# Storm-Tarran/LPR_381_Group_V22

Measured on AMD Instinct MI355X. Metric: simplex pivots/sec on 4096x8192 fp64 tableau; % HBM roofline, higher is better.
Workload: dtype f64

## Files before the change

### lpr_381_group_v22_amd/csrc/engine_common.hpp

```cpp
#pragma once

#include <hip/hip_runtime.h>

#include <cfloat>
#include <cstdint>
#include <cstdio>
#include <cstring>
#include <string>
#include <vector>

#include "../../include/lpr_engine.h"

#pragma clang fp contract(off)

namespace lpr {

constexpr int kWave = 64;
constexpr int kLdAlign = 16;
constexpr int32_t kRunning = -100;
constexpr int kMaxHeadGroups = 32;

void set_error(const char* fmt, ...);
const char* get_error();

#define LPR_HIP(expr)                                                                     \
    do {                                                                                  \
        hipError_t _e = (expr);                                                           \
        if (_e != hipSuccess) {                                                           \
            ::lpr::set_error("%s failed: %s (%s:%d)", #expr, hipGetErrorString(_e),       \
                             __FILE__, __LINE__);                                         \
            return LPR_DEVICE_ERROR;                                                      \
        }                                                                                 \
    } while (0)

// ... 117 lines not shown
    bool poisoned = false;
    hipGraphExec_t graph = nullptr;
    int graph_batch = 0;
    int graph_variant = -1;
    struct GraphKey {
        const void *T = nullptr, *T2 = nullptr, *log = nullptr, *basis = nullptr;
        const void *next_col = nullptr, *colbuf = nullptr;
        int rows = 0, cols = 0, ld = 0;
        bool operator==(const GraphKey& o) const {
            return T == o.T && T2 == o.T2 && log == o.log && basis == o.basis &&
                   next_col == o.next_col && colbuf == o.colbuf && rows == o.rows &&
                   cols == o.cols && ld == o.ld;
        }
    } graph_key;
    void* ov = nullptr;
    void* cut = nullptr;
    void* small = nullptr;
};

namespace lpr {
int tableau_reserve_rows(lpr_tableau* t, int rows_needed);
}
```

### lpr_381_group_v22_amd/csrc/lpr_engine.hip

```cpp
#include "engine_common.hpp"

#include <cmath>
#include <cstdlib>

#include <cstdarg>
#include <new>

#pragma clang fp contract(off)

namespace lpr {

static thread_local std::string g_err;

void set_error(const char* fmt, ...) {
    char buf[1024];
    va_list ap;
    va_start(ap, fmt);
    vsnprintf(buf, sizeof buf, fmt, ap);
    va_end(ap);
    g_err = buf;
}
const char* get_error() { return g_err.c_str(); }

void launch_select(lpr_tableau* t, int mode, int e_in, int r_in, int32_t* out_i);
// ... 24 lines not shown
int ov2_begin(lpr_tableau* t);
int ov2_launch_step(lpr_tableau* t, int K, int tr, int lp, int flags, hipEvent_t ev_start,
                    hipEvent_t ev_stop, int snap_slot);
int ov_read_stamps(lpr_tableau* t, uint64_t* out, int64_t cap, int64_t* count);
int ov2_join(lpr_tableau* t);
void ov_launch_sweep(lpr_tableau* t, int tr);
struct OvPoll {
    int32_t status, pending, kdone, cur, error;
    int64_t applied;
    double z[2];
};
int ov_poll(lpr_tableau* t, int parity, bool with_flags, OvPoll* out);
int ov_snapshot(lpr_tableau* t, int slot);
int ov_snapshot_wait(lpr_tableau* t, int slot, OvPoll* out);
void ov_adopt_buffer(lpr_tableau* t, int cur);
void rev_orphan(lpr_revised* s);
void bb_orphan(lpr_bb* b);
void sens_orphan(lpr_sens* s);
void comm_orphan(lpr_comm* c);
void knap_orphan(lpr_knap* k);
void batch_orphan(lpr_batch* b);
void bb_batch_orphan(lpr_bb_batch* b);
void sens_batch_orphan(lpr_sens_batch* b);
void cut_batch_orphan(lpr_cut_batch* b);
void knap_batch_orphan(lpr_knap_batch* b);
void rev_batch_orphan(lpr_rev_batch* b);
}
void lpr_cut_release(lpr_tableau* t);
namespace lpr {

// ... 135 lines not shown
    return t->graph && t->graph_batch == batch && t->graph_variant == variant &&
           t->graph_key == graph_key_now(t);
}

static void graph_stamp(lpr_tableau* t, int batch, int variant) {
    t->graph_batch = batch;
    t->graph_variant = variant;
    t->graph_key = graph_key_now(t);
}

static void release_device(lpr_tableau* t) {
    hipSetDevice(t->eng->device);
    if (t->eng->stream) hipStreamSynchronize(t->eng->stream);
    drop_graph(t);
    lpr_cut_release(t);
    ov_release(t);
    small_release(t);
    for (hipEvent_t ev : t->ev) hipEventDestroy(ev);
    t->ev.clear();
    hipFree(t->T);
    hipFree(t->T2);
    hipFree(t->rowbuf);
    hipFree(t->colbuf);
    hipFree(t->next_col);
    hipFree(t->next_rhs);
    hipFree(t->zparts);
    hipFree(t->basis);
    hipFree(t->log);
    hipFree(t->state);
    hipFree(t->scratch_i);
// ... 425 lines not shown
                if (q != hipErrorNotReady) LPR_HIP(q);
                (void)hipGetLastError();
            }
        }
        rc = drain();
        if (rc != LPR_OK_OPTIMAL) return rc;
    }
    ov_adopt_buffer(t, pl.cur);
    t->total_pivots = applied;
    res->status = status;
    res->block = K;
    res->pivots = applied - start_iter;
    res->total_pivots = applied;
    res->z = pl.z[applied & 1];
    return status;
}

}

using namespace lpr;

#define LPR_LIVE(t)                                                              \
    do {                                                                         \
        if (!(t) || !(t)->eng) {                                                 \
            set_error("tableau handle is null or its engine has been closed");   \
            return LPR_BAD_ARGUMENT;                                             \
        }                                                                        \
        if ((t)->poisoned) {                                                     \
            set_error("tableau handle is unusable: an earlier solve ended in a " \
                      "device-side hand-off timeout");                           \
// ... 228 lines not shown
    if (ld) *ld = t->ld;
    return LPR_OK_OPTIMAL;
}


int lpr_primal_solve(lpr_tableau* t, const lpr_solve_opts* opts, lpr_solve_result* res) {
    LPR_LIVE(t);
    if (!t || !res) {
        set_error("lpr_primal_solve: null argument");
        return LPR_BAD_ARGUMENT;
    }
    lpr_solve_opts o;
    std::memset(&o, 0, sizeof o);
    if (opts) o = *opts;
    const int hflags = (o.variant >> 16) & 511;
    o.variant &= 0xffff;
    if ((o.variant & 0xff00) == 0x5000) o.variant = 0x3000 | (o.variant & 0xff);
    if ((o.variant & 0xff00) == 0x6000) o.variant = 0x4000 | (o.variant & 0xff);
    lpr_engine* e = t->eng;
    hipStream_t s = e->stream;
    LPR_HIP(hipSetDevice(e->device));

    if (use_small(t, o)) return solve_small(t, o, res);
    if (use_fused(t, o)) return solve_fused(t, o, res);
    {
        const int K = block_size(t, o);
        if (K > 1) {
            const size_t tbytes = (size_t)t->rows * t->ld * sizeof(double);
            const bool big = (o.variant & 0xff00) == 0 && tbytes > kOverlapBytes;
            bool two_streams = (o.variant & 0xff00) == 0x3000 || big;
            const int tr = (o.variant & 0xff00) ? (o.variant & 0xff) : 8;
            if (two_streams && ov_ensure(t, true) != LPR_OK_OPTIMAL) two_streams = false;
            return solve_overlapped(t, o, K, tr, two_streams, hflags, res);
        }
    }
    const int variant = (o.variant > 0 && o.variant < 0x7000) ? o.variant - 1 : default_variant(t);
    int batch = o.batch > 0 ? o.batch : default_batch(t);
    const bool timed = o.time_kernels != 0;
    const int64_t start_iter = t->total_pivots;
    const int64_t max_iter = o.max_pivots > 0 ? start_iter + o.max_pivots : 0;

    PivotState* hs = t->h_state;
    hs->status = kRunning;
    hs->iter = start_iter;
    hs->max_iter = max_iter;
    hs->log_cap = t->log_cap;
    LPR_HIP(hipMemcpyAsync(&t->state->status, &hs->status, sizeof(int32_t), hipMemcpyHostToDevice,
// ... 250 lines not shown
```

### lpr_381_group_v22_amd/csrc/overlap_kernels.hip

```cpp
#include "engine_common.hpp"
#include "select_common.hpp"

#include <new>

#include <hip/hip_ext.h>

#pragma clang fp contract(off)

#ifndef LPR_OV_DIAG
#define LPR_OV_DIAG 0
#endif

namespace lpr {

constexpr int kOvMax = 16;
constexpr int kOvNT = 256;
constexpr int kOvGroups = 64;
constexpr unsigned kOvSpinMax = 1u << 22;
constexpr int kOvDoneCopies = 32;
constexpr int kOvDoneStride = 1088;
constexpr size_t kOvFlagWords = (size_t)(kOvDoneCopies + 1) * kOvDoneStride;
#ifndef LPR_OV_TILE_ROWS
#define LPR_OV_TILE_ROWS 32
#endif
// ... 10 lines not shown
#endif
constexpr bool kOvWaveHandoff = LPR_OV_WAVE_HANDOFF != 0;
constexpr int kOvWPG = kOvNT / 64;
constexpr int kOvParts = kOvGroups * kOvWPG;

struct OvCtl {
    int32_t status;
    int32_t pending;
    int32_t kdone;
    int32_t slot;
    int32_t cur;
    int32_t sweep;
    int32_t r[kOvMax];
    int32_t error;
    int32_t head_xcc;
    int64_t staged;
    int64_t applied;
    int64_t max_iter;
    int64_t log_cap;
};

struct OvBuffers {
    double* Tb[2];
    double* prow;
    double* fcol;
    double* zrow;
    double* bvec;
    ZPart* zparts;
    double* rparts;
    unsigned long long* gran;
    unsigned long long* xgran;
    unsigned long long* hx;
    unsigned* tileq;
    unsigned* sflag;
    unsigned long long* dbg;
    OvCtl* ctl;
    unsigned* bar;
    int32_t* basis;
    int32_t* log;
};

constexpr int kOvStampsPerPivot = 12;
constexpr int kOvStampPivots = 64;
constexpr size_t kOvDbgLaunch = (size_t)kOvStampPivots * kOvStampsPerPivot + 8;
constexpr size_t kOvDbgWords = kOvDbgLaunch + 64;

__global__ __launch_bounds__(1024) void k_ov_prologue(const double* __restrict__ T, int ld, int R,
                                                      int C, double* __restrict__ zrow,
                                                      double* __restrict__ bvec0,
                                                      ZPart* __restrict__ bank, int G,
                                                      unsigned long long* gbank,
                                                      unsigned epoch,
                                                      unsigned long long* gran_all,
                                                      unsigned long long* __restrict__ xgran,
                                                      unsigned* __restrict__ bar,
                                                      unsigned* __restrict__ tileq,
                                                      unsigned long long* __restrict__ hx,
                                                      unsigned* __restrict__ sflag) {
    __shared__ double lds_v[16];
    __shared__ int lds_i[16];
    const int tid = threadIdx.x, nt = blockDim.x;
    for (int k = tid; k < 9 * kOvParts; k += nt) gran_all[k] = 0ull;
    for (int k = tid; k < kOvGroups; k += nt) xgran[k] = 0ull;
    if (tid < 4) bar[tid] = 0u;
    if (tid < 2) tileq[tid] = 0u;
    if (tid == 0) *hx = 0ull;
    if (tid < 4) sflag[tid] = 0u;
    if (tid < kOvDoneCopies) sflag[(size_t)(tid + 1) * kOvDoneStride] = 0u;
    __syncthreads();
    Cand c;
    c.v = 0.0;
    c.i = -1;
    for (int j = tid; j < ld; j += nt) {
        const double v = T[j];
        zrow[j] = v;
        if (j < C - 1 && v < c.v) {
            c.v = v;
            c.i = j;
        }
    }
    c = block_cand_min(c, lds_v, lds_i);
    if (tid < G) {
        const double v = (tid == 0) ? c.v : 0.0;
        const int i = (tid == 0) ? c.i : -1;
        bank[tid].v = v;
        bank[tid].i = i;
    }
    const int nparts = kOvWaveHandoff ? G * kOvWPG : G;
    if (tid < nparts) {
        const double v = (tid == 0) ? c.v : 0.0;
        const int i = (tid == 0) ? c.i : -1;
        const unsigned long long e = (unsigned long long)epoch << 32;
        gbank[tid * 3 + 0] = e | (unsigned)__double2loint(v);
// ... 181 lines not shown
    __syncthreads();
    if (threadIdx.x == 0) {
        Cand r;
        r.v = lds_v[0];
        r.i = lds_i[0];
        for (int w = 1; w < (int)blockDim.x / kWave; ++w) {
            Cand o;
            o.v = lds_v[w];
            o.i = lds_i[w];
            r = cand_min(r, o);
        }
        gr_publish(g3, epoch, r.v, r.i, l2);
    }
}

template <int NT, bool STAMP>
__device__ void ov_heads(const OvBuffers B, int ld, int R, int C, int Rp, int K, int G, int lp,
                         bool solo, int spread, int no_l2, int wait_sweeps, int heads_done = -1) {
    if ((int)blockIdx.x % spread != 0) return;
    __shared__ double lds_v[16];
    __shared__ int lds_i[16];
    __shared__ int s_pick[2];
    const int tid = threadIdx.x, nt = blockDim.x;
    const int g = (int)blockIdx.x / spread;
    const bool lead = (g == 0);
    const OvCtl* ci = B.ctl + lp;
    OvCtl* co = B.ctl + (lp ^ 1);
    const int32_t status = ci->status;
    const int32_t pend_in = ci->pending;
    const int kb = solo ? 0 : ci->kdone;
    const int sa = ci->slot;
// ... 27 lines not shown
    double2* zrow2 = reinterpret_cast<double2*>(B.zrow);

    const int i_first = g * nt + tid, c2_first = g * nt + tid;
    const bool have_i = i_first < R, have_c = c2_first < ld2;
    double fA[kOvMax], myf[kOvMax];
    double2 pA[kOvMax], myp[kOvMax];
#pragma unroll
    for (int t = 0; t < kOvMax; ++t) {
        fA[t] = (t < kb && have_i) ? fcolA[(size_t)t * Rp + i_first] : 0.0;
        pA[t] = (t < kb && have_c) ? prowA2[(size_t)t * ld2 + c2_first] : make_double2(0.0, 0.0);
        myf[t] = 0.0;
        myp[t] = make_double2(0.0, 0.0);
    }
    double2 myz = have_c ? zrow2[c2_first] : make_double2(0.0, 0.0);
    double myb = have_i ? B.bvec[(size_t)(staged0 & 1) * Rp + i_first] : 0.0;
    const int lane = tid & (kWave - 1);
    const int rAv = (lane < kb) ? ci->r[lane] : -1;
    int rNv = -1;
    unsigned maskA = 0u, maskN = 0u;
#pragma unroll
    for (int t = 0; t < kOvMax; ++t) {
        const int rt = __builtin_amdgcn_readlane(rAv, t);
        maskA |= (have_i && rt == i_first) ? (1u << t) : 0u;
    }

    int32_t pend_out = pend_in;
    int32_t status_out = status;
    int count = 0;
    int err = 0;
    bool l2 = false;
// ... 84 lines not shown
                        s_pick[1] = fail;
                    }
                }
                __syncthreads();
                e = s_pick[0];
                if (s_pick[1]) {
                    err = 1;
                    break;
                }
            }
            OV_STAMP(q, 1);
            if (e < 0) {
                pend_out = LPR_OK_OPTIMAL;
                break;
            }
            double cq = have_i ? Tin[(size_t)i_first * ld + e] : 0.0;
            double pv = 0.0;
            if (lane < kb) pv = prowA[(size_t)lane * ld + e];
            else if (lane >= kOvMax && lane - kOvMax < q - 1)
                pv = xld(&prowN[(size_t)(lane - kOvMax) * ld + e]);
            if (STAMP) {
                __builtin_amdgcn_s_waitcnt(0);
                OV_STAMP(q, 2);
                OV_STAMP(q, 3);
            }
#pragma unroll
            for (int t = 0; t < kOvMax; ++t) {
                const double pt = ov_rl(pv, t);
                const double prod = fA[t] * pt;
                const double d = cq - prod;
                cq = ov_bitsel(maskA, t, pt, d);
            }
#pragma unroll
            for (int t = 0; t < kOvMax; ++t) {
                const double pt = ov_rl(pv, kOvMax + t);
                const double prod = myf[t] * pt;
                const double d = cq - prod;
                cq = ov_bitsel(maskN, t, pt, d);
            }
#pragma unroll
            for (int t = 0; t < kOvMax; ++t)
                if (t == q - 1) myf[t] = cq;
            Cand rc;
            rc.v = DBL_MAX;
            rc.i = -1;
            if (have_i) {
                hst(&colq[i_first], cq, l2);
                if (i_first >= 1 && cq > 1e-9) {
                    const double ratio = ieee_div(myb, cq);
                    if (ratio >= 0 && ratio < DBL_MAX) {
                        rc.v = ratio;
                        rc.i = i_first;
                    }
                }
            }
            for (int i = i_first + G * nt; i < R; i += G * nt) {
                double c = Tin[(size_t)i * ld + e];
#pragma unroll
                for (int t = 0; t < kOvMax; ++t) {
                    if (t < kb) {
// ... 7 lines not shown
                    }
                }
#pragma unroll
                for (int t = 0; t < kOvMax; ++t) {
                    if (t < q - 1) {
                        const double pt = ov_rl(pv, kOvMax + t);
                        if (i == __builtin_amdgcn_readlane(rNv, t)) {
                            c = pt;
                        } else {
                            const double prod = fcolN[(size_t)t * Rp + i] * pt;
                            c = c - prod;
                        }
                    }
                }
                hst(&colq[i], c, l2);
                if (c > 1e-9) {
                    const double ratio = ieee_div(bprev[i], c);
                    if (ratio >= 0 && ratio < rc.v) {
                        rc.v = ratio;
                        rc.i = i;
                    }
                }
            }
            OV_STAMP(q, 4);
            OV_STAMP(q, 5);
            int r;
            if (kOvWaveHandoff) {
                ov_publish_wave_min(rc, B.gran + ((size_t)2 * kOvParts + g * kOvWPG + tid / kWave) * 3,
                                    (unsigned)(2 * pidx + 2), l2);
                OV_STAMP(q, 6);
                int fail = 0;
                const Cand rr = gr_collect_waves(B.gran + (size_t)2 * 3 * kOvParts, G * kOvWPG,
                                                 (unsigned)(2 * pidx + 2), DBL_MAX, &fail);
                r = rr.i;
                if (fail) {
                    err = 1;
                    break;
                }
            } else {
                ov_publish_min(rc, lds_v, lds_i, B.gran + (size_t)(2 * kOvParts + g) * 3,
// ... 23 lines not shown
            if (mx > 0 && pidx >= mx) {
                pend_out = LPR_PIVOT_LIMIT;
                break;
            }

            double2 w = have_c ? Tin2[(size_t)r * ld2 + c2_first] : make_double2(0.0, 0.0);
            double fv = 0.0;
            {
                const double* src = nullptr;
                if (lane < kb) src = fcolA + (size_t)lane * Rp + r;
                else if (lane >= kOvMax && lane - kOvMax < q - 1)
                    src = fcolN + (size_t)(lane - kOvMax) * Rp + r;
                else if (lane == 32) src = bprev + r;
                else if (lane == 33) src = colq + r;
                else if (lane == 34) src = colq;
                if (src) fv = xld(src);
            }
            if (STAMP) {
                __builtin_amdgcn_s_waitcnt(0);
                OV_STAMP(q, 8);
            }
            const double wr = ov_rl(fv, 32);
            const double p = ov_rl(fv, 33);
            const double f0 = ov_rl(fv, 34);
            const unsigned ra = (unsigned)__ballot(lane < kb && rAv == r);
            const unsigned rn = (unsigned)__ballot(lane < q - 1 && rNv == r);
            if ((ra | rn) == 0u) {
#pragma unroll
                for (int t = 0; t < kOvMax; ++t) {
                    const double f = ov_rl(fv, t);
                    const double px = f * pA[t].x;
// ... 22 lines not shown
                        w.y = w.y - py;
                    }
                }
#pragma unroll
                for (int t = 0; t < kOvMax; ++t) {
                    if ((rn >> t) & 1u) {
                        w = myp[t];
                    } else {
                        const double f = ov_rl(fv, kOvMax + t);
                        const double px = f * myp[t].x;
                        const double py = f * myp[t].y;
                        w.x = w.x - px;
                        w.y = w.y - py;
                    }
                }
            }
            double dq[3];
            {
                const double dn[3] = {wr, w.x, w.y}, dd[3] = {p, p, p};
                ieee_div_n<3>(dn, dd, dq);
            }
            const double prhs = dq[0];
            if (lane == q - 1) rNv = r;
            if (have_i && i_first == r) maskN |= 1u << (q - 1);
            Cand n;
            n.v = 0.0;
            n.i = -1;
            if (have_c) {
                const int j = 2 * c2_first;
                double2 pq;
                pq.x = (j < C) ? dq[1] : 0.0;
                pq.y = (j + 1 < C) ? dq[2] : 0.0;
#pragma unroll
                for (int t = 0; t < kOvMax; ++t)
                    if (t == q - 1) myp[t] = pq;
                hst(&prowN[(size_t)(q - 1) * ld + j], pq.x, l2);
                hst(&prowN[(size_t)(q - 1) * ld + j + 1], pq.y, l2);
                const double mxp = f0 * pq.x;
                const double myp2 = f0 * pq.y;
                myz.x = myz.x - mxp;
                myz.y = myz.y - myp2;
                zrow2[c2_first] = myz;
                if (j < C - 1 && myz.x < n.v) {
                    n.v = myz.x;
                    n.i = j;
                }
                if (j + 1 < C - 1 && myz.y < n.v) {
                    n.v = myz.y;
                    n.i = j + 1;
                }
            }
            for (int c2 = c2_first + G * nt; c2 < ld2; c2 += G * nt) {
                double2 ww = Tin2[(size_t)r * ld2 + c2];
                double2 z = zrow2[c2];
#pragma unroll
                for (int t = 0; t < kOvMax; ++t) {
                    if (t < kb) {
                        const double2 ps = prowA2[(size_t)t * ld2 + c2];
                        if ((ra >> t) & 1u) {
                            ww = ps;
                        } else {
                            const double f = ov_rl(fv, t);
                            const double px = f * ps.x;
                            const double py = f * ps.y;
// ... 39 lines not shown
                    n.i = j + 1;
                }
            }
            if (have_i) {
                const double prod = cq * prhs;
                myb = (i_first == r) ? prhs : myb - prod;
                hst(&bnew[i_first], myb, l2);
            }
            for (int i = i_first + G * nt; i < R; i += G * nt) {
                const double prod = colq[i] * prhs;
                hst(&bnew[i], (i == r) ? prhs : bprev[i] - prod, l2);
            }
            OV_STAMP(q, 9);
            if (lead && tid == 0) {
                co->r[q - 1] = r;
                B.basis[r - 1] = e;
                if (pidx < log_cap) {
                    B.log[2 * pidx] = r;
                    B.log[2 * pidx + 1] = e;
                }
            }
            count = q;
            OV_STAMP(q, 10);
            if (kOvWaveHandoff)
                ov_publish_wave_min(n, B.gran + ((size_t)((pidx + 1) & 1) * kOvParts + g * kOvWPG +
                                                 tid / kWave) * 3,
                                    (unsigned)(2 * (pidx + 1) + 1), l2 && q < K);
            else
                ov_publish_min(n, lds_v, lds_i,
                               B.gran + ((size_t)((pidx + 1) & 1) * kOvParts + g) * 3,
                               (unsigned)(2 * (pidx + 1) + 1), l2 && q < K);
            OV_STAMP(q, 11);
        }
    }
#undef OV_STAMP
// ... 9 lines not shown
                    err = 1;
                    break;
                }
                __builtin_amdgcn_s_sleep(2);
            }
        }
        co->status = err ? LPR_DEVICE_ERROR : status_out;
        co->pending = pend_out;
        co->kdone = staged_now ? count : 0;
        co->slot = staged_now ? (sa ^ 1) : sa;
        co->staged = staged0 + (staged_now ? count : 0);
        co->max_iter = mx;
        co->log_cap = log_cap;
        co->error = err | ci->error;
        co->head_xcc = l2 ? (int)my_xcc : (staging ? -1 : ci->head_xcc);
        B.bar[lp ^ 1] = 0u;
        if (wait_sweeps >= 0) {
            const int ks = (status == kRunning) ? ci->kdone : 0;
            co->applied = ci->applied + ks;
            co->cur = (ks > 0) ? (ci->cur ^ 1) : ci->cur;
            co->sweep = ci->sweep ^ (ks > 0 ? 1 : 0);
        }
        if (solo) {
            B.tileq[1] = 0u;
            co->applied = ci->applied;
            co->cur = ci->cur;
            co->sweep = ci->sweep;
        }
    }
    if (heads_done >= 0) {
// ... 305 lines not shown
            co->applied = ci->applied + K;
            co->cur = (K > 0 && !INPLACE) ? (cur ^ 1) : cur;
            co->sweep = ci->sweep ^ (K > 0 ? 1 : 0);
        }
        B.tileq[lp ^ 1] = 0u;
        if (INPLACE) {
            co->status = ci->status;
            co->pending = ci->pending;
            co->kdone = 0;
            co->slot = ci->slot;
            co->staged = ci->staged;
            co->max_iter = ci->max_iter;
            co->log_cap = ci->log_cap;
            co->error = ci->error;
            co->head_xcc = ci->head_xcc;
            B.bar[lp ^ 1] = 0u;
        }
    }
    if (K <= 0) return;
    const int sa = ci->slot;
    const double* __restrict__ fc = fcol + (size_t)sa * kOvMax * Rp;
    const ov_v2d* __restrict__ prow2 =
        reinterpret_cast<const ov_v2d*>(prow + (size_t)sa * kOvMax * ld);
    if (static_tile >= 0) {
        ov_one_tile<TR, DB, INPLACE, TROWS>(B, ci, fc, prow2, static_tile, ld, R, Rp, K, cur);
        return;
    }
    const int ld2 = ld >> 1;
    const int nct = (ld2 + kOvNT - 1) / kOvNT, nrt = (R + TROWS - 1) / TROWS;
    const int ntiles = nct * nrt;
// ... 59 lines not shown
            const int pol = (at < ic_tiles ? 1 : 0) | (at >= ntiles - ic_tiles ? 2 : 0);
#define LPR_OV_HALF(P)                                                                             \
    ov_one_tile<TR, false, INPLACE, TROWS / 2, P>(B, ci, fc, prow2, tsplit + (u >> 1), ld, R, Rp, \
                                                  K, cur, TROWS, (u & 1) * (TROWS / 2))
            switch (pol) {
                case 1: LPR_OV_HALF(1); break;
                case 2: LPR_OV_HALF(2); break;
                case 3: LPR_OV_HALF(3); break;
                default: LPR_OV_HALF(0); break;
            }
#undef LPR_OV_HALF
        }
    }
}

template <int NT, bool STAMP>
__global__ __launch_bounds__(NT) void k_ov2_heads(const OvBuffers B, int ld, int R, int C, int Rp,
                                                  int K, int G, int lp, int spread, int no_l2,
                                                  int wait_sweeps, int heads_done) {
    ov_heads<NT, STAMP>(B, ld, R, C, Rp, K, G, lp, false, spread, no_l2, wait_sweeps, heads_done);
}

template <int TR, bool DB>
__global__ __launch_bounds__(kOvNT) void k_ov2_sweep(const OvBuffers B,
                                                     const double* __restrict__ fcol_ro,
                                                     const double* __restrict__ prow_ro, int ld,
                                                     int R, int Rp, int lp, int avoid,
                                                     int write_ctl, int sweeps_done,
                                                     int wait_heads, int hint_xcc, int ic_tiles,
                                                     int tall_pairs) {
    ov_tiles<TR, DB, false>(B, fcol_ro, prow_ro, ld, R, Rp, lp, -1, avoid, write_ctl != 0,
                            sweeps_done, wait_heads, hint_xcc, ic_tiles, tall_pairs);
}

template <int NT, bool STAMP>
__global__ __launch_bounds__(NT) void k_ov_heads(const OvBuffers B, int ld, int R, int C, int Rp,
                                                 int K, int G, int spread, int no_l2) {
    ov_heads<NT, STAMP>(B, ld, R, C, Rp, K, G, 0, true, spread, no_l2, -1);
}

template <int TR, bool DB, int TROWS = kOvTileRows>
__global__ __launch_bounds__(kOvNT) void k_ov_sweep(const OvBuffers B,
                                                    const double* __restrict__ fcol_ro,
                                                    const double* __restrict__ prow_ro, int ld,
                                                    int R, int Rp) {
    ov_tiles<TR, DB, true, TROWS>(B, fcol_ro, prow_ro, ld, R, Rp, 1, (int)blockIdx.x, 0);
}

}

#ifndef LPR_OV_KERNELS_ONLY

struct lpr_overlap_ctx {
    int rows = 0, ld = 0, Rp = 0;
    lpr::OvBuffers b{};
    lpr::OvCtl* h_ctl = nullptr;
    double* h_z = nullptr;
    double* T2 = nullptr;
    hipStream_t hstream = nullptr;
    hipEvent_t ev_h[2] = {nullptr, nullptr}, ev_s[2] = {nullptr, nullptr};
    int ev_idx = 0;
// ... 148 lines not shown
    std::memset(h, 0, 2 * sizeof(OvCtl));
    h[0].status = kRunning;
    h[0].pending = kRunning;
    h[0].staged = iter;
    h[0].applied = iter;
    h[0].max_iter = max_iter;
    h[0].log_cap = t->log_cap;
    h[0].head_xcc = -1;
    h[0].sweep = c->sweep_dir;
    h[1] = h[0];
    LPR_HIP(hipMemcpyAsync(c->b.ctl, h, 2 * sizeof(OvCtl), hipMemcpyHostToDevice, s));
    hipLaunchKernelGGL(k_ov_prologue, dim3(1), dim3(1024), 0, s, t->T, t->ld, t->rows, t->cols,
                       c->b.zrow, c->b.bvec + (size_t)(iter & 1) * c->Rp,
                       c->b.zparts + (iter & 1) * kOvGroups, ov_groups(t),
                       c->b.gran + (size_t)(iter & 1) * 3 * kOvParts, (unsigned)(2 * iter + 1),
                       c->b.gran, c->b.xgran, c->b.bar, c->b.tileq, c->b.hx, c->b.sflag);
    LPR_HIP(hipGetLastError());
    return LPR_OK_OPTIMAL;
}

int ov_set_log(lpr_tableau* t, int parity) {
    lpr_overlap_ctx* c = static_cast<lpr_overlap_ctx*>(t->ov);
    c->b.log = t->log;
    c->h_ctl[0].log_cap = t->log_cap;
    LPR_HIP(hipMemcpyAsync(&c->b.ctl[parity].log_cap, &c->h_ctl[0].log_cap, sizeof(int64_t),
                           hipMemcpyHostToDevice, t->eng->stream));
    LPR_HIP(hipStreamSynchronize(t->eng->stream));
    return LPR_OK_OPTIMAL;
}

void ov_launch_heads(lpr_tableau* t, int K, int flags) {
// ... 56 lines not shown
    const bool by_event = (flags & 32) == 0;
    const int wait_sweeps = by_event ? -1 : c->steps;
    const bool sweep_dev = (flags & 64) != 0 && !c->batch_first && c->steps >= 2 &&
                           c->head_xcc_hint >= 0 && snap_slot < 0;
    const int heads_done = (flags & 64) ? c->steps + 1 : -1;
    if (by_event) LPR_HIP(hipStreamWaitEvent(H, c->last_sweep, 0));
    if (!sweep_dev) LPR_HIP(hipStreamWaitEvent(S, c->ev_h[prev], 0));
    if (snap_slot >= 0) {
        LPR_HIP(hipMemcpyAsync(&c->h_snap[snap_slot], &c->b.ctl[lp], sizeof(OvCtl),
                               hipMemcpyDeviceToHost, S));
        LPR_HIP(hipEventRecord(c->ev_snap[snap_slot], S));
    }
    const int G = ov_groups(t);
    const int spread = ov_spread(G, flags);
    const int no_l2 = (flags & 6) ? 1 : 0;
    if (flags & 1)
        hipExtLaunchKernelGGL((k_ov2_heads<kOvNT, true>), dim3(G * spread), dim3(kOvNT), 0, H,
                              nullptr, c->ev_h[cur], 0, c->b, t->ld, t->rows, t->cols, c->Rp, K, G,
                              lp, spread, no_l2, wait_sweeps, heads_done);
    else
        hipExtLaunchKernelGGL((k_ov2_heads<kOvNT, false>), dim3(G * spread), dim3(kOvNT), 0, H,
                              nullptr, c->ev_h[cur], 0, c->b, t->ld, t->rows, t->cols, c->Rp, K, G,
                              lp, spread, no_l2, wait_sweeps, heads_done);
    const int nct = (t->ld / 2 + kOvNT - 1) / kOvNT;
    const int nrt = (t->rows + kOvTileRows - 1) / kOvTileRows;
    const dim3 grid(ov_sweep_grid(t, nct * nrt)), blk(kOvNT);
    const int avoid = (flags & (2 | 4 | 8)) ? 0 : ((flags & 16) ? 1 : 2);
    hipEvent_t sweep_done = ev_stop ? ev_stop : c->ev_s[cur];
    const int ic_tiles =
        (flags & 128) ? 0 : (int)(((size_t)kOvIcMB << 20) / ((size_t)kOvTileRows * kOvNT * 16));
    const int tall_pairs = (flags & 256) ? 0 : nrt * LPR_OV_TALL_PCT / 200;
// ... 87 lines not shown
        LPR_HIP(hipStreamSynchronize(t->eng->stream));
        LPR_HIP(hipMemcpy(out, c->b.dbg, (size_t)n * sizeof(uint64_t), hipMemcpyDeviceToHost));
    }
    return LPR_OK_OPTIMAL;
}

void ov_adopt_buffer(lpr_tableau* t, int cur) {
    lpr_overlap_ctx* c = static_cast<lpr_overlap_ctx*>(t->ov);
    if (cur == 1) {
        double* tmp = t->T;
        t->T = c->T2;
        c->T2 = tmp;
    }
}

}
#endif
```

Baseline: 98250.

## Run simplex on a condensed tableau that drops basic columns and uses spare slots

```diff
diff --git a/lpr_381_group_v22_amd/csrc/engine_common.hpp b/lpr_381_group_v22_amd/csrc/engine_common.hpp
--- a/lpr_381_group_v22_amd/csrc/engine_common.hpp
+++ b/lpr_381_group_v22_amd/csrc/engine_common.hpp
@@ -18,6 +18,8 @@
 constexpr int kWave = 64;
 constexpr int kLdAlign = 16;
 constexpr int32_t kRunning = -100;
+constexpr int32_t kOvLeaveNonFinite = -101;
+constexpr int32_t kOvLeaveSpares = -102;
 constexpr int kMaxHeadGroups = 32;
 
 void set_error(const char* fmt, ...);
@@ -165,6 +167,7 @@
         }
     } graph_key;
     void* ov = nullptr;
+    void* ovc = nullptr;
     void* cut = nullptr;
     void* small = nullptr;
 };
diff --git a/lpr_381_group_v22_amd/csrc/lpr_engine.hip b/lpr_381_group_v22_amd/csrc/lpr_engine.hip
--- a/lpr_381_group_v22_amd/csrc/lpr_engine.hip
+++ b/lpr_381_group_v22_amd/csrc/lpr_engine.hip
@@ -62,6 +62,14 @@
 int ov_snapshot(lpr_tableau* t, int slot);
 int ov_snapshot_wait(lpr_tableau* t, int slot, OvPoll* out);
 void ov_adopt_buffer(lpr_tableau* t, int cur);
+void ovc_release(lpr_tableau* t);
+bool ovc_fits(const lpr_tableau* t, int spares);
+int ovc_width(const lpr_tableau* t, int spares);
+int ovc_ensure(lpr_tableau* t, int spares);
+int ovc_condense(lpr_tableau* t, bool* ok);
+void ovc_enter(lpr_tableau* t);
+void ovc_leave(lpr_tableau* t);
+int ovc_expand(lpr_tableau* t);
 void rev_orphan(lpr_revised* s);
 void bb_orphan(lpr_bb* b);
 void sens_orphan(lpr_sens* s);
@@ -227,6 +235,7 @@
     if (t->eng->stream) hipStreamSynchronize(t->eng->stream);
     drop_graph(t);
     lpr_cut_release(t);
+    ovc_release(t);
     ov_release(t);
     small_release(t);
     for (hipEvent_t ev : t->ev) hipEventDestroy(ev);
@@ -682,6 +691,61 @@
     res->total_pivots = applied;
     res->z = pl.z[applied & 1];
     return status;
+}
+
+static constexpr int64_t kOvcMinPivots = 1024;
+
+static int ovc_spares(const lpr_tableau* t) {
+    if (const char* sp = std::getenv("LPR_TEST_OV_SPARES")) {
+        const long v = std::strtol(sp, nullptr, 10);
+        if (v >= 1 && v <= 4096) return (int)v;
+    }
+    const int s = (t->rows - 1) / 8 - 1;
+    return s < 1 ? 1 : s;
+}
+
+static bool use_condensed(const lpr_tableau* t, const lpr_solve_opts& o, int cflags, int hflags) {
+    if (cflags & 1) return false;
+    if (hflags & (1 | 32 | 64)) return false;
+    const int S = ovc_spares(t);
+    if (!ovc_fits(t, S)) return false;
+    if (cflags & 2) return true;
+    if (o.max_pivots > 0 && o.max_pivots < kOvcMinPivots) return false;
+    return ovc_width(t, S) < t->ld;
+}
+
+static int solve_condensed(lpr_tableau* t, const lpr_solve_opts& o, int K, int tr, int hflags,
+                           lpr_solve_result* res) {
+    const int64_t first = t->total_pivots;
+    lpr_solve_opts oc = o;
+    for (;;) {
+        const int64_t done = t->total_pivots - first;
+        if (o.max_pivots > 0) oc.max_pivots = o.max_pivots - done;
+        bool ok = false;
+        int rc = ovc_ensure(t, ovc_spares(t));
+        if (rc == LPR_OK_OPTIMAL) rc = ovc_condense(t, &ok);
+        if (rc != LPR_OK_OPTIMAL && rc != LPR_OUT_OF_MEMORY) return rc;
+        int status;
+        if (rc != LPR_OK_OPTIMAL || !ok) {
+            status = solve_overlapped(t, oc, K, tr, true, hflags, res);
+        } else {
+            ovc_enter(t);
+            status = solve_overlapped(t, oc, K, tr, true, hflags, res);
+            ovc_leave(t);
+            if (status == LPR_DEVICE_ERROR || status == LPR_OUT_OF_MEMORY ||
+                status == LPR_BAD_ARGUMENT)
+                return status;
+            rc = ovc_expand(t);
+            if (rc != LPR_OK_OPTIMAL) return rc;
+            if (status == kOvLeaveSpares) continue;
+            if (status == kOvLeaveNonFinite) {
+                if (o.max_pivots > 0) oc.max_pivots = o.max_pivots - (t->total_pivots - first);
+                status = solve_overlapped(t, oc, K, tr, true, hflags, res);
+            }
+        }
+        res->pivots = t->total_pivots - first;
+        return status;
+    }
 }
 
 }
@@ -940,6 +1004,7 @@
     std::memset(&o, 0, sizeof o);
     if (opts) o = *opts;
     const int hflags = (o.variant >> 16) & 511;
+    const int cflags = (o.variant >> 25) & 3;
     o.variant &= 0xffff;
     if ((o.variant & 0xff00) == 0x5000) o.variant = 0x3000 | (o.variant & 0xff);
     if ((o.variant & 0xff00) == 0x6000) o.variant = 0x4000 | (o.variant & 0xff);
@@ -957,6 +1022,13 @@
             bool two_streams = (o.variant & 0xff00) == 0x3000 || big;
             const int tr = (o.variant & 0xff00) ? (o.variant & 0xff) : 8;
             if (two_streams && ov_ensure(t, true) != LPR_OK_OPTIMAL) two_streams = false;
+            if (two_streams && (big || (cflags & 2)) && !(cflags & 1) &&
+                ovc_fits(t, ovc_spares(t)) && ovc_width(t, ovc_spares(t)) < t->ld) {
+                const int er = ovc_ensure(t, ovc_spares(t));
+                if (er != LPR_OK_OPTIMAL && er != LPR_OUT_OF_MEMORY) return er;
+            }
+            if (two_streams && use_condensed(t, o, cflags, hflags))
+                return solve_condensed(t, o, K, tr, hflags, res);
             return solve_overlapped(t, o, K, tr, two_streams, hflags, res);
         }
     }
diff --git a/lpr_381_group_v22_amd/csrc/overlap_kernels.hip b/lpr_381_group_v22_amd/csrc/overlap_kernels.hip
--- a/lpr_381_group_v22_amd/csrc/overlap_kernels.hip
+++ b/lpr_381_group_v22_amd/csrc/overlap_kernels.hip
@@ -48,6 +48,8 @@
     int32_t r[kOvMax];
     int32_t error;
     int32_t head_xcc;
+    int32_t spares;
+    int32_t pad_;
     int64_t staged;
     int64_t applied;
     int64_t max_iter;
@@ -72,6 +74,10 @@
     unsigned* bar;
     int32_t* basis;
     int32_t* log;
+    int32_t* colid;
+    unsigned long long* rowvar;
+    unsigned long long* cstate;
+    int spare0, nspare;
 };
 
 constexpr int kOvStampsPerPivot = 12;
@@ -90,7 +96,8 @@
                                                       unsigned* __restrict__ bar,
                                                       unsigned* __restrict__ tileq,
                                                       unsigned long long* __restrict__ hx,
-                                                      unsigned* __restrict__ sflag) {
+                                                      unsigned* __restrict__ sflag,
+                                                      const int32_t* __restrict__ colid) {
     __shared__ double lds_v[16];
     __shared__ int lds_i[16];
     const int tid = threadIdx.x, nt = blockDim.x;
@@ -110,7 +117,7 @@
         zrow[j] = v;
         if (j < C - 1 && v < c.v) {
             c.v = v;
-            c.i = j;
+            c.i = colid ? ((colid[j] << 16) | j) : j;
         }
     }
     c = block_cand_min(c, lds_v, lds_i);
@@ -322,7 +329,7 @@
     }
 }
 
-template <int NT, bool STAMP>
+template <int NT, bool STAMP, bool COND = false>
 __device__ void ov_heads(const OvBuffers B, int ld, int R, int C, int Rp, int K, int G, int lp,
                          bool solo, int spread, int no_l2, int wait_sweeps, int heads_done = -1) {
     if ((int)blockIdx.x % spread != 0) return;
@@ -380,6 +387,14 @@
     }
     double2 myz = have_c ? zrow2[c2_first] : make_double2(0.0, 0.0);
     double myb = have_i ? B.bvec[(size_t)(staged0 & 1) * Rp + i_first] : 0.0;
+    int idx = -1, idy = -1, used = 0;
+    if (COND) {
+        if (have_c) {
+            idx = B.colid[2 * c2_first];
+            idy = B.colid[2 * c2_first + 1];
+        }
+        used = ci->spares;
+    }
     const int lane = tid & (kWave - 1);
     const int rAv = (lane < kb) ? ci->r[lane] : -1;
     int rNv = -1;
@@ -494,6 +509,8 @@
                 pend_out = LPR_OK_OPTIMAL;
                 break;
             }
+            const int e_id = COND ? (e >> 16) : e;
+            if (COND) e &= 0xffff;
             double cq = have_i ? Tin[(size_t)i_first * ld + e] : 0.0;
             double pv = 0.0;
             if (lane < kb) pv = prowA[(size_t)lane * ld + e];
@@ -524,6 +541,7 @@
             Cand rc;
             rc.v = DBL_MAX;
             rc.i = -1;
+            bool badf = COND && have_i && !(fabs(cq) <= DBL_MAX);
             if (have_i) {
                 hst(&colq[i_first], cq, l2);
                 if (i_first >= 1 && cq > 1e-9) {
@@ -561,6 +579,7 @@
                     }
                 }
                 hst(&colq[i], c, l2);
+                if (COND && !(fabs(c) <= DBL_MAX)) badf = true;
                 if (c > 1e-9) {
                     const double ratio = ieee_div(bprev[i], c);
                     if (ratio >= 0 && ratio < rc.v) {
@@ -571,6 +590,8 @@
             }
             OV_STAMP(q, 4);
             OV_STAMP(q, 5);
+            if (COND && badf)
+                __hip_atomic_store(B.cstate, 1ull, __ATOMIC_RELAXED, __HIP_MEMORY_SCOPE_AGENT);
             int r;
             if (kOvWaveHandoff) {
                 ov_publish_wave_min(rc, B.gran + ((size_t)2 * kOvParts + g * kOvWPG + tid / kWave) * 3,
@@ -624,7 +645,28 @@
                 else if (lane == 32) src = bprev + r;
                 else if (lane == 33) src = colq + r;
                 else if (lane == 34) src = colq;
+                else if (COND && lane == 35) src = reinterpret_cast<const double*>(B.cstate);
+                else if (COND && lane == 36)
+                    src = reinterpret_cast<const double*>(B.rowvar + (r - 1));
                 if (src) fv = xld(src);
+            }
+            int sigma = -1;
+            int leave_id = -1;
+            if (COND) {
+                if (__double2loint(ov_rl(fv, 35)) != 0) {
+                    pend_out = kOvLeaveNonFinite;
+                    break;
+                }
+                const double lv = ov_rl(fv, 36);
+                if (__double2loint(lv) < 0) {
+                    if (used >= B.nspare) {
+                        pend_out = kOvLeaveSpares;
+                        break;
+                    }
+                    sigma = B.spare0 + used;
+                    leave_id = __double2hiint(lv);
+                    used += 1;
+                }
             }
             if (STAMP) {
                 __builtin_amdgcn_s_waitcnt(0);
@@ -677,6 +719,16 @@
                         w.y = w.y - py;
                     }
                 }
+            }
+            if (COND && sigma >= 0 && have_c && (sigma >> 1) == c2_first) {
+                if (sigma & 1) {
+                    w.y = 1.0;
+                    idy = leave_id;
+                } else {
+                    w.x = 1.0;
+                    idx = leave_id;
+                }
+                B.colid[sigma] = leave_id;
             }
             double dq[3];
             {
@@ -704,13 +756,23 @@
                 myz.x = myz.x - mxp;
                 myz.y = myz.y - myp2;
                 zrow2[c2_first] = myz;
-                if (j < C - 1 && myz.x < n.v) {
-                    n.v = myz.x;
-                    n.i = j;
-                }
-                if (j + 1 < C - 1 && myz.y < n.v) {
-                    n.v = myz.y;
-                    n.i = j + 1;
+                if (COND) {
+                    Cand a, b;
+                    a.v = myz.x;
+                    a.i = (j < C - 1 && myz.x < 0.0) ? ((idx << 16) | j) : -1;
+                    b.v = myz.y;
+                    b.i = (j + 1 < C - 1 && myz.y < 0.0) ? ((idy << 16) | (j + 1)) : -1;
+                    const Cand m = ov_cand_min_sel(a, b);
+                    if (m.i >= 0) n = m;
+                } else {
+                    if (j < C - 1 && myz.x < n.v) {
+                        n.v = myz.x;
+                        n.i = j;
+                    }
+                    if (j + 1 < C - 1 && myz.y < n.v) {
+                        n.v = myz.y;
+                        n.i = j + 1;
+                    }
                 }
             }
             for (int c2 = c2_first + G * nt; c2 < ld2; c2 += G * nt) {
@@ -780,11 +842,14 @@
             OV_STAMP(q, 9);
             if (lead && tid == 0) {
                 co->r[q - 1] = r;
-                B.basis[r - 1] = e;
+                B.basis[r - 1] = e_id;
                 if (pidx < log_cap) {
                     B.log[2 * pidx] = r;
-                    B.log[2 * pidx + 1] = e;
-                }
+                    B.log[2 * pidx + 1] = e_id;
+                }
+                if (COND)
+                    hst(B.rowvar + (r - 1),
+                        ((unsigned long long)(unsigned)e_id << 32) | (unsigned)e, l2);
             }
             count = q;
             OV_STAMP(q, 10);
@@ -824,6 +889,8 @@
         co->log_cap = log_cap;
         co->error = err | ci->error;
         co->head_xcc = l2 ? (int)my_xcc : (staging ? -1 : ci->head_xcc);
+        co->spares = used;
+        co->pad_ = 0;
         B.bar[lp ^ 1] = 0u;
         if (wait_sweeps >= 0) {
             const int ks = (status == kRunning) ? ci->kdone : 0;
@@ -1159,6 +1226,8 @@
             co->log_cap = ci->log_cap;
             co->error = ci->error;
             co->head_xcc = ci->head_xcc;
+            co->spares = ci->spares;
+            co->pad_ = 0;
             B.bar[lp ^ 1] = 0u;
         }
     }
@@ -1248,11 +1317,11 @@
     }
 }
 
-template <int NT, bool STAMP>
+template <int NT, bool STAMP, bool COND = false>
 __global__ __launch_bounds__(NT) void k_ov2_heads(const OvBuffers B, int ld, int R, int C, int Rp,
                                                   int K, int G, int lp, int spread, int no_l2,
                                                   int wait_sweeps, int heads_done) {
-    ov_heads<NT, STAMP>(B, ld, R, C, Rp, K, G, lp, false, spread, no_l2, wait_sweeps, heads_done);
+    ov_heads<NT, STAMP, COND>(B, ld, R, C, Rp, K, G, lp, false, spread, no_l2, wait_sweeps, heads_done);
 }
 
 template <int TR, bool DB>
@@ -1279,6 +1348,137 @@
                                                     const double* __restrict__ prow_ro, int ld,
                                                     int R, int Rp) {
     ov_tiles<TR, DB, true, TROWS>(B, fcol_ro, prow_ro, ld, R, Rp, 1, (int)blockIdx.x, 0);
+}
+
+__global__ __launch_bounds__(1024) void k_ov_cond_map(const int32_t* __restrict__ basis, int R,
+                                                      int C, int Wc, int Wp,
+                                                      int32_t* __restrict__ rowof,
+                                                      int32_t* __restrict__ slotof,
+                                                      int32_t* __restrict__ colid,
+                                                      unsigned long long* __restrict__ rowvar,
+                                                      unsigned long long* __restrict__ cstate,
+                                                      unsigned* __restrict__ fail) {
+    __shared__ int s_cnt[1024];
+    const int tid = threadIdx.x, nt = blockDim.x;
+    for (int j = tid; j < C; j += nt) rowof[j] = 0;
+    for (int s = tid; s < Wp; s += nt) colid[s] = -1;
+    if (tid == 0) {
+        cstate[0] = 0ull;
+        fail[0] = 0u;
+    }
+    __syncthreads();
+    for (int i = 1 + tid; i < R; i += nt) {
+        const int b = basis[i - 1];
+        if (b < 0 || b >= C - 1) {
+            fail[0] = 1u;
+        } else {
+            if (atomicExch(&rowof[b], i) != 0) fail[0] = 1u;
+            rowvar[i - 1] = ((unsigned long long)(unsigned)b << 32) | 0xffffffffull;
+        }
+    }
+    __syncthreads();
+    const int per = (C - 1 + nt - 1) / nt;
+    const int j0 = min(tid * per, C - 1), j1 = min(j0 + per, C - 1);
+    int cnt = 0;
+    for (int j = j0; j < j1; ++j) cnt += (rowof[j] == 0) ? 1 : 0;
+    s_cnt[tid] = cnt;
+    __syncthreads();
+    if (tid == 0) {
+        int acc = 0;
+        for (int k = 0; k < nt; ++k) {
+            const int c = s_cnt[k];
+            s_cnt[k] = acc;
+            acc += c;
+        }
+        if (acc != C - R) fail[0] = 1u;
+        slotof[C - 1] = Wc - 1;
+        colid[Wc - 1] = C - 1;
+    }
+    __syncthreads();
+    int s = s_cnt[tid];
+    for (int j = j0; j < j1; ++j) {
+        if (rowof[j] == 0) {
+            if (s < Wc - 1) colid[s] = j;
+            slotof[j] = s++;
+        } else {
+            slotof[j] = -1;
+        }
+    }
+}
+
+__global__ __launch_bounds__(256) void k_ov_condense(const double* __restrict__ T, int ld, int C,
+                                                     double* __restrict__ Tc, int Wp, int Wc,
+                                                     int nres, const int32_t* __restrict__ slotof,
+                                                     const int32_t* __restrict__ rowof,
+                                                     unsigned* __restrict__ fail) {
+    if (fail[0]) return;
+    const int k = blockIdx.y;
+    const int j0 = 2 * (blockIdx.x * blockDim.x + threadIdx.x);
+    if (j0 < ld) {
+        if (j0 >= C) return;
+        const ov_v2d v2 = __builtin_nontemporal_load(
+            reinterpret_cast<const ov_v2d*>(&T[(size_t)k * ld + j0]));
+#pragma unroll
+        for (int h = 0; h < 2; ++h) {
+            const int j = j0 + h;
+            if (j >= C) break;
+            const double v = h ? v2.y : v2.x;
+            const int s = slotof[j];
+            if (s >= 0) {
+                if (s < Wp) Tc[(size_t)k * Wp + s] = v;
+            } else {
+                const long long want = (rowof[j] == k) ? 0x3ff0000000000000ll : 0ll;
+                if (__double_as_longlong(v) != want) fail[1] = 1u;
+            }
+        }
+    } else {
+#pragma unroll
+        for (int h = 0; h < 2; ++h) {
+            const int s = nres + (j0 + h - ld);
+            if (s < Wp && s != Wc - 1) Tc[(size_t)k * Wp + s] = 0.0;
+        }
+    }
+}
+
+__global__ __launch_bounds__(1024) void k_ov_expand_map(int R, int C, int Wp,
+                                                        const int32_t* __restrict__ colid,
+                                                        const unsigned long long* __restrict__ rowvar,
+                                                        int32_t* __restrict__ rowof,
+                                                        int32_t* __restrict__ slotof) {
+    const int tid = threadIdx.x, nt = blockDim.x;
+    for (int j = tid; j < C; j += nt) {
+        rowof[j] = 0;
+        slotof[j] = -1;
+    }
+    __syncthreads();
+    for (int s = tid; s < Wp; s += nt) {
+        const int id = colid[s];
+        if (id >= 0 && id < C) slotof[id] = s;
+    }
+    for (int i = 1 + tid; i < R; i += nt) {
+        const unsigned long long rv = rowvar[i - 1];
+        if ((int)(unsigned)rv < 0) rowof[(int)(rv >> 32)] = i;
+    }
+}
+
+__global__ __launch_bounds__(256) void k_ov_expand(const double* __restrict__ Tc, int Wp,
+                                                   double* __restrict__ T, int ld, int C,
+                                                   const int32_t* __restrict__ slotof,
+                                                   const int32_t* __restrict__ rowof) {
+    const int k = blockIdx.y;
+    const int j0 = 2 * (blockIdx.x * blockDim.x + threadIdx.x);
+    if (j0 >= ld) return;
+    double v[2] = {0.0, 0.0};
+#pragma unroll
+    for (int h = 0; h < 2; ++h) {
+        const int j = j0 + h;
+        if (j < C) {
+            const int s = slotof[j];
+            if (s >= 0) v[h] = __builtin_nontemporal_load(&Tc[(size_t)k * Wp + s]);
+            else if (k > 0 && rowof[j] == k) v[h] = 1.0;
+        }
+    }
+    *reinterpret_cast<ov_v2d*>(&T[(size_t)k * ld + j0]) = ov_v2d{v[0], v[1]};
 }
 
 }
@@ -1457,7 +1657,8 @@
                        c->b.zrow, c->b.bvec + (size_t)(iter & 1) * c->Rp,
                        c->b.zparts + (iter & 1) * kOvGroups, ov_groups(t),
                        c->b.gran + (size_t)(iter & 1) * 3 * kOvParts, (unsigned)(2 * iter + 1),
-                       c->b.gran, c->b.xgran, c->b.bar, c->b.tileq, c->b.hx, c->b.sflag);
+                       c->b.gran, c->b.xgran, c->b.bar, c->b.tileq, c->b.hx, c->b.sflag,
+                       (const int32_t*)c->b.colid);
     LPR_HIP(hipGetLastError());
     return LPR_OK_OPTIMAL;
 }
@@ -1544,7 +1745,11 @@
     const int G = ov_groups(t);
     const int spread = ov_spread(G, flags);
     const int no_l2 = (flags & 6) ? 1 : 0;
-    if (flags & 1)
+    if (c->b.colid)
+        hipExtLaunchKernelGGL((k_ov2_heads<kOvNT, false, true>), dim3(G * spread), dim3(kOvNT), 0,
+                              H, nullptr, c->ev_h[cur], 0, c->b, t->ld, t->rows, t->cols, c->Rp, K,
+                              G, lp, spread, no_l2, wait_sweeps, heads_done);
+    else if (flags & 1)
         hipExtLaunchKernelGGL((k_ov2_heads<kOvNT, true>), dim3(G * spread), dim3(kOvNT), 0, H,
                               nullptr, c->ev_h[cur], 0, c->b, t->ld, t->rows, t->cols, c->Rp, K, G,
                               lp, spread, no_l2, wait_sweeps, heads_done);
@@ -1662,5 +1867,145 @@
     }
 }
 
+struct OvcCtx {
+    int rows = 0, cols = 0, ld = 0, spares = 0;
+    int nres = 0, Wc = 0, Wp = 0;
+    void* ov = nullptr;
+    double* Tc = nullptr;
+    int32_t *colid = nullptr, *slotof = nullptr, *rowof = nullptr;
+    unsigned long long *rowvar = nullptr, *cstate = nullptr;
+    unsigned *fail = nullptr, *h_fail = nullptr;
+    double* T_full = nullptr;
+    int ld_full = 0, cols_full = 0;
+    void* ov_full = nullptr;
+};
+
+void ovc_release(lpr_tableau* t) {
+    OvcCtx* x = static_cast<OvcCtx*>(t->ovc);
+    if (!x) return;
+    void* keep = t->ov;
+    t->ov = x->ov;
+    ov_release(t);
+    t->ov = keep;
+    hipFree(x->Tc);
+    hipFree(x->colid);
+    hipFree(x->slotof);
+    hipFree(x->rowof);
+    hipFree(x->rowvar);
+    hipFree(x->cstate);
+    hipFree(x->fail);
+    if (x->h_fail) hipHostFree(x->h_fail);
+    delete x;
+    t->ovc = nullptr;
+}
+
+bool ovc_fits(const lpr_tableau* t, int spares) {
+    const int nres = t->cols - t->rows;
+    if (t->rows < 2 || nres < 1 || spares < 1) return false;
+    if (t->cols > 32767) return false;
+    const long Wp = align_up(nres + spares + 1, kLdAlign);
+    return Wp <= 32767 && Wp / 2 <= (long)kOvGroups * kOvNT;
+}
+
+int ovc_width(const lpr_tableau* t, int spares) {
+    return align_up(t->cols - t->rows + spares + 1, kLdAlign);
+}
+
+void ovc_enter(lpr_tableau* t) {
+    OvcCtx* x = static_cast<OvcCtx*>(t->ovc);
+    x->T_full = t->T;
+    x->ld_full = t->ld;
+    x->cols_full = t->cols;
+    x->ov_full = t->ov;
+    t->T = x->Tc;
+    t->ld = x->Wp;
+    t->cols = x->Wc;
+    t->ov = x->ov;
+    x->Tc = nullptr;
+}
+
+void ovc_leave(lpr_tableau* t) {
+    OvcCtx* x = static_cast<OvcCtx*>(t->ovc);
+    x->Tc = t->T;
+    x->ov = t->ov;
+    t->T = x->T_full;
+    t->ld = x->ld_full;
+    t->cols = x->cols_full;
+    t->ov = x->ov_full;
+}
+
+int ovc_ensure(lpr_tableau* t, int spares) {
+    OvcCtx* x = static_cast<OvcCtx*>(t->ovc);
+    if (x && x->rows == t->rows && x->cols == t->cols && x->ld == t->ld && x->spares == spares)
+        return LPR_OK_OPTIMAL;
+    ovc_release(t);
+    x = new (std::nothrow) OvcCtx();
+    if (!x) return LPR_OUT_OF_MEMORY;
+    x->rows = t->rows;
+    x->cols = t->cols;
+    x->ld = t->ld;
+    x->spares = spares;
+    x->nres = t->cols - t->rows;
+    x->Wc = x->nres + spares + 1;
+    x->Wp = align_up(x->Wc, kLdAlign);
+    t->ovc = x;
+    hipError_t err = hipSuccess;
+    auto chk = [&](hipError_t e) { if (err == hipSuccess) err = e; };
+    chk(hipMalloc(&x->Tc, (size_t)t->rows * x->Wp * sizeof(double)));
+    chk(hipMalloc(&x->colid, (size_t)x->Wp * sizeof(int32_t)));
+    chk(hipMalloc(&x->slotof, (size_t)t->cols * sizeof(int32_t)));
+    chk(hipMalloc(&x->rowof, (size_t)t->cols * sizeof(int32_t)));
+    chk(hipMalloc(&x->rowvar, (size_t)t->rows * sizeof(unsigned long long)));
+    chk(hipMalloc(&x->cstate, 2 * sizeof(unsigned long long)));
+    chk(hipMalloc(&x->fail, 2 * sizeof(unsigned)));
+    chk(hipHostMalloc(&x->h_fail, 2 * sizeof(unsigned)));
+    int rc = LPR_OK_OPTIMAL;
+    if (err != hipSuccess) {
+        (void)hipGetLastError();
+        rc = err == hipErrorOutOfMemory ? LPR_OUT_OF_MEMORY : LPR_DEVICE_ERROR;
+    } else {
+        ovc_enter(t);
+        t->ov = nullptr;
+        rc = ov_ensure(t, true);
+        if (rc == LPR_OK_OPTIMAL) {
+            lpr_overlap_ctx* c = static_cast<lpr_overlap_ctx*>(t->ov);
+            c->b.colid = x->colid;
+            c->b.rowvar = x->rowvar;
+            c->b.cstate = x->cstate;
+            c->b.spare0 = x->nres;
+            c->b.nspare = spares;
+        }
+        ovc_leave(t);
+    }
+    if (rc != LPR_OK_OPTIMAL) ovc_release(t);
+    return rc;
+}
+
+int ovc_condense(lpr_tableau* t, bool* ok) {
+    OvcCtx* x = static_cast<OvcCtx*>(t->ovc);
+    hipStream_t s = t->eng->stream;
+    hipLaunchKernelGGL(k_ov_cond_map, dim3(1), dim3(1024), 0, s, t->basis, t->rows, t->cols, x->Wc,
+                       x->Wp, x->rowof, x->slotof, x->colid, x->rowvar, x->cstate, x->fail);
+    const int span = (t->ld + (x->Wp - x->nres) + 1) / 2;
+    hipLaunchKernelGGL(k_ov_condense, dim3((span + 255) / 256, t->rows), dim3(256), 0, s, t->T,
+                       t->ld, t->cols, x->Tc, x->Wp, x->Wc, x->nres, x->slotof, x->rowof, x->fail);
+    LPR_HIP(hipGetLastError());
+    LPR_HIP(hipMemcpyAsync(x->h_fail, x->fail, 2 * sizeof(unsigned), hipMemcpyDeviceToHost, s));
+    LPR_HIP(hipStreamSynchronize(s));
+    *ok = x->h_fail[0] == 0u && x->h_fail[1] == 0u;
+    return LPR_OK_OPTIMAL;
+}
+
+int ovc_expand(lpr_tableau* t) {
+    OvcCtx* x = static_cast<OvcCtx*>(t->ovc);
+    hipStream_t s = t->eng->stream;
+    hipLaunchKernelGGL(k_ov_expand_map, dim3(1), dim3(1024), 0, s, t->rows, t->cols, x->Wp,
+                       x->colid, x->rowvar, x->rowof, x->slotof);
+    hipLaunchKernelGGL(k_ov_expand, dim3((t->ld / 2 + 255) / 256, t->rows), dim3(256), 0, s, x->Tc,
+                       x->Wp, t->T, t->ld, t->cols, x->slotof, x->rowof);
+    LPR_HIP(hipGetLastError());
+    return LPR_OK_OPTIMAL;
+}
+
 }
 #endif
```

After: 105,300 (median of 6 runs). +7.2%, better.
